# kxhit/vMAP

Measured on AMD Instinct MI355X. Metric: training rays/sec (all objects) per step, higher is better.
Workload: dtype f32 I/O, masters, accumulation; matrix operands split into bf16 planes: forward 6 products (~2^-24, float32-equivalent), backward 3 (~2^-16)

## Files before the change

### vmap_amd/csrc/k_s32.hip

```cpp
#include "launch.h"
#include "split_kernels.h"

namespace vl {

namespace {
template <bool BWD, bool MULTI, bool STAMPS, bool W3, bool B6 = false, bool PV = false, bool OL = false>
int main_v(const vk::StepArgs& a, hipStream_t st) {
    auto kern = vk::step_main_s32<BWD, MULTI, STAMPS, W3, B6, PV, OL>;
    if (int rc = ensure_dynamic_lds(reinterpret_cast<const void*>(kern), vk::Img32s::LDS_BYTES, "step_main_s32")) return rc;
    const int grid = a.xcd_affine ? 8 * ((a.n_obj + 7) / 8) * a.NW : a.n_obj * a.NW;
    VL_LAUNCH_MAIN(kern, dim3(grid), dim3(vk::kWG), vk::Img32s::LDS_BYTES, st, a);
    return launched("step_main_s32");
}
#ifdef VMAPSTEP_AB
template <bool MULTI, bool W3, bool B6>
int main_of(const vk::StepArgs& a, hipStream_t st) {
    auto kern = vk::step_main_s32_of<MULTI, W3, B6>;
    if (int rc = ensure_dynamic_lds(reinterpret_cast<const void*>(kern), vk::Img32s::LDS_BYTES, "step_main_s32")) return rc;
    const int grid = a.xcd_affine ? 8 * ((a.n_obj + 7) / 8) * a.NW : a.n_obj * a.NW;
    VL_LAUNCH_MAIN(kern, dim3(grid), dim3(vk::kWG), vk::Img32s::LDS_BYTES, st, a);
    return launched("step_main_s32");
}
template <bool MULTI, bool STAMPS, bool W3, bool B6>
int main_ob(const vk::StepArgs& a, hipStream_t st) {
    auto kern = vk::step_main_s32_ob<MULTI, STAMPS, W3, B6>;
    if (int rc = ensure_dynamic_lds(reinterpret_cast<const void*>(kern), vk::Img32s::LDS_BYTES, "step_main_s32")) return rc;
    const int grid = a.xcd_affine ? 8 * ((a.n_obj + 7) / 8) * a.NW : a.n_obj * a.NW;
    VL_LAUNCH_MAIN(kern, dim3(grid), dim3(vk::kWG), vk::Img32s::LDS_BYTES, st, a);
    return launched("step_main_s32");
}
#endif
template <bool BWD, bool STAMPS>
int main_bs(const vk::StepArgs& a, hipStream_t st) {
    const bool multi = a.NW < a.NG;
#ifdef VMAPSTEP_AB
    if (a.ab_flags & 8) {
        if constexpr (BWD) {
            if (!(a.ab_flags & 7)) {
                if constexpr (STAMPS) {
                    if (!a.weights_bf16 && !a.bwd6 && !multi) return main_ob<false, true, true, false>(a, st);
                } else {
                    if (a.weights_bf16) return multi ? main_ob<true, false, false, false>(a, st) : main_ob<false, false, false, false>(a, st);
                    if (a.bwd6) return multi ? main_ob<true, false, true, true>(a, st) : main_ob<false, false, true, true>(a, st);
                    return multi ? main_ob<true, false, true, false>(a, st) : main_ob<false, false, true, false>(a, st);
                }
            }
        }
        return fail(-2, "tuning.ws_flags bit 6 (the former backward of step_main_s32): training steps without bit 3, 4 or 5; phase stamps with float32 weights, the three-product backward and one pass per workgroup only");
    }
    if (a.ab_flags & 4) {
        if constexpr (BWD && !STAMPS) {
            if (!(a.ab_flags & 3)) {
                if (a.weights_bf16) return multi ? main_of<true, false, false>(a, st) : main_of<false, false, false>(a, st);
                if (a.bwd6) return multi ? main_of<true, true, true>(a, st) : main_of<false, true, true>(a, st);
                return multi ? main_of<true, true, false>(a, st) : main_of<false, true, false>(a, st);
            }
        }
        return fail(-2, "tuning.ws_flags bit 5 (the former front of step_main_s32): training steps without phase stamps, bit 3 or bit 4");
    }
    if (a.ab_flags & 2) {
        if constexpr (BWD && !STAMPS) {
            if (!a.bwd6 && !(a.ab_flags & 1)) {
                if (a.weights_bf16) return multi ? main_v<true, true, false, false, false, false, true>(a, st) : main_v<true, false, false, false, false, false, true>(a, st);
                return multi ? main_v<true, true, false, true, false, false, true>(a, st) : main_v<true, false, false, true, false, false, true>(a, st);
            }
        }
        return fail(-2, "tuning.ws_flags bit 4 (the former load order of step_main_s32): training steps without phase stamps, bit 3 or the six-product backward");
    }
// ... 36 lines not shown
```

### vmap_amd/csrc/split_kernels.h

```cpp
#pragma once
#ifndef VS_ABL
#define VS_ABL 0
#endif
#include "step_kernels.h"
#include "wave_reduce.h"
#ifndef VS_FRONT_PARTS
#define VS_FRONT_PARTS 15
#endif
#ifndef VS_BACK_PARTS
#define VS_BACK_PARTS 7
#endif

#ifndef VS_ABL
#define VS_ABL 0
#endif
#if VS_ABL & 2
#define VS_BWD_BARRIER() do { } while (0)
#else
#define VS_BWD_BARRIER() __syncthreads()
#endif

namespace vk {

using wv::u32x2;
using wv::u32x4;

struct Img32s {
    static constexpr int PIT_IN = 208, PIT_M = 80, PIT_CAT = 272, PIT_C = 176;
    static constexpr int O_IN = 0, O_M1 = O_IN + 32 * PIT_IN, O_CAT = O_M1 + 32 * PIT_M, O_M2 = O_CAT + 32 * PIT_CAT,
                         O_C = O_M2 + 32 * PIT_M, PLANE = O_C + 32 * PIT_C;
    static constexpr int P_HI = 0, P_MID = PLANE, SMALL = 2 * PLANE, SMALL_BYTES = 2048, P_LO = SMALL + SMALL_BYTES,
                         END = P_LO + PLANE, BYTES = (END + 4095) / 4096 * 4096;
    static constexpr int ROUNDS = BYTES / 4096;
    static constexpr int ELEMS = PLANE / 2;
    static constexpr int B_M1 = 0, B_M2 = 32, W_A = 64, W_OC = 96, B_A = 192, B_OC = 196, PE_B = 200, SMALL_N = 208;
    static constexpr int G_PEB = SMALL_N, VEC_N = SMALL_N + 66 + 6;
    static constexpr int TILE = 32 * Lds32::TP * 4;
    static constexpr int TPL = TILE / 2;
    static constexpr int TPIT = 72;
    static constexpr int SCR = BYTES;
    static constexpr int STG = SCR;
    static constexpr int STG_BYTES = 2 * kWaves * TILE, kWavesTiles = kWaves * 2 * TILE;
    static constexpr int VEC = SCR + kWaves * 2 * TILE;
// ... 683 lines not shown
            } else {
                const unsigned pm = wv::pack_bf16(wv::after(ra[i], accB[0]), rb[i]);
                hm[i] = pm;
                hl[i] = wv::pack_bf16(ra[i] - bf_lo(pm), rb[i] - bf_hi(pm));
            }
        }
        wv::sched_fence();
    }
}

template <bool BIG>
__device__ __forceinline__ void octave_sincos(float a0, float (&s)[6], float (&c)[6]) {
    if (BIG) sincosf(a0, &s[0], &c[0]);
    else sincos_f32(a0, s[0], c[0]);
#pragma unroll
    for (int f = 1; f < 6; ++f) {
        const float t = s[f - 1] + s[f - 1];
        s[f] = t * c[f - 1];
        c[f] = fmaf(-t, s[f - 1], 1.0f);
    }
}

__device__ __forceinline__ void stage_put_s(float* stage, const f32x16& acc, int wave, int p31, int hi) {
    if (!(VS_ABL & 9)) stage_put(stage, acc, wave, p31, hi);
    else if (VS_ABL & 8) {
#pragma unroll
        for (int r = 0; r < 16; ++r) asm volatile("" ::"v"(acc[r]));
    }
}
__device__ __forceinline__ void stage_get_s(float (&q)[4], const float* stage, int wave, int p31, int hi) {
    if (!(VS_ABL & 9)) stage_get(q, stage, wave, p31, hi);
}

template <bool BWD, bool MULTI, bool STAMPS, bool W3, bool B6 = false, bool PV = false, bool OL = false, bool OF = false, bool OB = false>
__device__ __forceinline__ void step_main_s32_body(const StepArgs& a) {
    static_assert(!B6 || (W3 && BWD), "six-product backward: float32 weights, training instantiations");
    constexpr int OLD = OL ? 7 : VS_LOADS_OLD;
    constexpr int FP = OF ? 0 : VS_FRONT_PARTS;
    constexpr int BP = OB ? 0 : VS_BACK_PARTS;
    constexpr bool TC = (BP & 1) != 0, TD = (BP & 2) != 0, ZC = (BP & 4) != 0 && !MULTI;
    using I = Img32s;
    using F = Flat32;
    constexpr int H = 32;
    char* lds = reinterpret_cast<char*>(wv::lds_base());
    const char* W = lds;
    const float* SM = reinterpret_cast<const float*>(lds + I::SMALL);
    const int tid = threadIdx.x, lane = tid & 63, wave = tid >> 6, p31 = lane & 31, hi = lane >> 5;
    float* Gv = reinterpret_cast<float*>(lds + I::VEC) + wave * I::VEC_N;
    int obj, wgo;
    if (a.xcd_affine) {
        const int slot = blockIdx.x >> 3;
        const int og = slot / a.NW;
        obj = og * 8 + (blockIdx.x & 7);
        wgo = slot - og * a.NW;
        if (obj >= a.n_obj) return;
    } else {
        obj = blockIdx.x / a.NW;
        wgo = blockIdx.x - obj * a.NW;
    }
    unsigned* tmark = STAMPS && a.timing ? a.timing + ((long long)blockIdx.x * kWaves + wave) * kMarks : nullptr;
#define VS_MARK(i) do { if constexpr (STAMPS) { if (tmark && lane == 0) tmark[i] = wv::clock32(); } } while (0)
    VS_MARK(0);
    if (BWD) {
        for (int i = tid; i < kWaves * I::VEC_N; i += kWG) reinterpret_cast<float*>(lds + I::VEC)[i] = 0.0f;
    }
    float* loss_cells = reinterpret_cast<float*>(lds + I::LOSS);
    if (tid < kWaves * 4) loss_cells[tid] = 0.0f;
    float* out = a.part_grad + ((long long)(obj * a.NW + wgo)) * a.PP;
    float qacc[12][4];
#pragma unroll
    for (int b = 0; b < 12; ++b) {
#pragma unroll
        for (int i = 0; i < 4; ++i) qacc[b][i] = 0.0f;
// ... 221 lines not shown
            row[2] = sigmoidf_acc(r1);
            row[3] = sigmoidf_acc(r2);
        }
        if (BWD) {
            toF_put(reinterpret_cast<float*>(scrX), h4, p31, hi);
            toF_put(reinterpret_cast<float*>(scrD), hc, p31, hi);
        }
    }
    VS_MARK(4);
    if (!(VS_ABL & 65536)) __syncthreads();
    VS_MARK(5);
    {
        const StepArgs& al = wv::kernarg_late(a);
        if constexpr (OLD & 2) {
        if (!(VS_ABL & 2048))
        composite_phase<BWD>(al, cb, loss_cells, obj, ray0, nrays, wave, lane, tid,
                             (VS_ABL & 1024) ? rays_meta : finish_ray_meta(al, obj, rays_meta));
        } else if (!(VS_ABL & 2048)) composite_phase<BWD>(al, cb, loss_cells, obj, ray0, nrays, wave, lane, tid, rays_meta);
    }
    if (!(VS_ABL & 65536)) __syncthreads();
    VS_MARK(6);
    if (BWD) {
    float d_raw, d_c0, d_c1, d_c2;
    {
        const float* row = cb + pt * 8;
        d_raw = row[0]; d_c0 = row[1]; d_c1 = row[2]; d_c2 = row[3];
    }
    constexpr int DM = !W3 ? 0 : B6 ? 2 : 1, NA = kDpropMM(DM), NPW = !W3 ? 1 : B6 ? 3 : 2, NPB = B6 ? 3 : 2, NDW = kDwMM(B6), NDB = kDwDbMM(B6);
    unsigned dF[24];
    float dproj[11];
#pragma unroll
    for (int i = 0; i < 11; ++i) dproj[i] = 0.0f;
    unsigned dch[8], dcm[8], dcl[8], d4h[8], d4m[8], d4l[8];
    {
        float h4F[16], hcF[16];
        toF_get(h4F, reinterpret_cast<const float*>(scrX), p31, hi);
        toF_get(hcF, reinterpret_cast<const float*>(scrD), p31, hi);
        float ga = 0.0f, g0 = 0.0f, g1 = 0.0f, g2 = 0.0f, sa = 0.0f, s0 = 0.0f, s1 = 0.0f, s2 = 0.0f;
#pragma unroll
        for (int r = 0; r < 16; ++r) {
            const float* row = cbw + (r + 16 * hi) * 8;
            const float da = row[0], q0 = row[1], q1 = row[2], q2 = row[3];
            ga = fmaf(da, h4F[r], ga);
            g0 = fmaf(q0, hcF[r], g0); g1 = fmaf(q1, hcF[r], g1); g2 = fmaf(q2, hcF[r], g2);
            sa += da; s0 += q0; s1 += q1; s2 += q2;
        }
        ga += wv::swap_half(ga); g0 += wv::swap_half(g0); g1 += wv::swap_half(g1); g2 += wv::swap_half(g2);
        sa += wv::swap_half(sa); s0 += wv::swap_half(s0); s1 += wv::swap_half(s1); s2 += wv::swap_half(s2);
        if (hi == 0) {
            if constexpr (ZC) {
                Gv[I::W_A + p31] = 0.0f + ga;
                Gv[I::W_OC + p31] = 0.0f + g0;
                Gv[I::W_OC + H + p31] = 0.0f + g1;
                Gv[I::W_OC + 2 * H + p31] = 0.0f + g2;
                if (p31 == 0) {
                    Gv[I::B_A] = 0.0f + sa;
                    Gv[I::B_OC + 0] = 0.0f + s0;
                    Gv[I::B_OC + 1] = 0.0f + s1;
                    Gv[I::B_OC + 2] = 0.0f + s2;
                }
            } else {
                Gv[I::W_A + p31] += ga;
                Gv[I::W_OC + p31] += g0;
                Gv[I::W_OC + H + p31] += g1;
                Gv[I::W_OC + 2 * H + p31] += g2;
                if (p31 == 0) {
                    Gv[I::B_A] += sa;
                    Gv[I::B_OC + 0] += s0;
                    Gv[I::B_OC + 1] += s1;
                    Gv[I::B_OC + 2] += s2;
                }
            }
        }
        float dcp[16];
#pragma unroll
        for (int r = 0; r < 16; ++r) {
            const int j = phi(r, hi);
            const float v = SM[I::W_OC + j] * d_c0 + SM[I::W_OC + H + j] * d_c1 + SM[I::W_OC + 2 * H + j] * d_c2;
            dcp[r] = wv::opaque(hc[r]) > 0.0f ? v : 0.0f;
        }
        split_planes<16, NPB>(dcp, dch, dcm, dcl);
    }
    f32x16 acc2, accb;
    FinState fs;
    unsigned wA[24], wB[24], xA[24], xB[24];
    unsigned d3h[8], d3m[8], d3l[8], d2h[8], d2m[8], d2l[8], d1h[8], d1m[8], d1l[8], dF3[24], dF1[24];
    const auto nothing = [](int) {};
    const auto dproj_add = [&](int d, float v, float c) {
        if constexpr (TD) { const float sum = dproj[d] + v * c; dproj[d] = wv::after(sum, sum); }
        else dproj[d] += v * c;
    };
#define VS_FIN(KIND, K, QI, STG, OW, OB, BLK, NC)                                                                             \
    [&](int i) {                                                                                                              \
        if (i == 0) fin_chunk<KIND, K, MULTI>(0, fs, qacc[QI], STG, OW, OB, BLK, NC, wave, p31, hi);                          \
        if (i == NA - 3) fin_chunk<KIND, K, MULTI>(1, fs, qacc[QI], STG, OW, OB, BLK, NC, wave, p31, hi);                     \
    }
    const SelOps SEL = sel_ops(p31, hi);
    wt_get<I::PIT_C, NPW>(wA, W + I::O_C, 0, TL);
    toF_mm3<4, NPB>(dF, dch, dcm, dcl, SEL);
    toF_mm3<4, NPB>(xA, h4h, h4m, h4l, SEL);
    wt_get<I::PIT_C, NPW>(wB, W + I::O_C, 2, TL);
#pragma unroll
    for (int r = 0; r < 16; ++r) acc2[r] = SM[I::W_A + phi(r, hi)] * d_raw;
    mm_dprop_il<DM>(acc2, wA, dch, dcm, dcl, nothing);
    toF_mm3<4, NPB>(xB, e2h, e2m, e2l, SEL);
    zero_acc(acc);
    mm_dw_il<false, B6>(acc, accb, dF, xA, [&](int i) {
#pragma unroll
        for (int j = i * 8 / NDW; j < (i + 1) * 8 / NDW; ++j) mask_split_pair<NPB>(j, acc2, h4h, d4h, d4m, d4l, acc[0]);
    });
    wt_get<I::PIT_C, NPW>(wA, W + I::O_C, 4, TL);
    VS_BWD_BARRIER();
    zero_acc(acc2);
    mm_dprop_il<DM>(acc2, wB, dch, dcm, dcl, [&](int i) { if (i == NA - 1) stage_put_s(stg0, acc, wave, p31, hi); });
    toF_mm3<2, NPB>(xA, e2h + 8, e2m + 8, e2l + 8, SEL);
    wt_get<I::PIT_M, NPW>(wB, W + I::O_M2, 0, TL);
    zero_acc(acc);
    mm_dw_il<false, B6>(acc, accb, dF, xB, [&](int i) {
        if (i < 4) {
#pragma unroll
            for (int r = 4 * i; r < 4 * i + 4; ++r) dproj_add(r >> 1, wv::after(acc2[r], acc[0]), cfac[r >> 1][4 + (r & 1)]);
        }
    });
    VS_BWD_BARRIER();
    zero_acc(acc2);
    {
        auto fin = VS_FIN(0, H + kEmb2, 0, stg0, out + F::W_C, nullptr, 0, 32);
        mm_dprop_il<DM>(acc2, wA, dch, dcm, dcl, [&](int i) { fin(i); if (i == NA - 1) stage_put_s(stg1, acc, wave, p31, hi); });
    }
    toF_mm3<4, NPB>(xB, h3h, h3m, h3l, SEL);
    wt_get<I::PIT_CAT, NPW>(wA, W + I::O_CAT, 0, TL);
    zero_acc(acc);
    mm_dw_il<false, B6>(acc, accb, dF, xA, [&](int i) {
        if (i < 3) {
#pragma unroll
            for (int r = 2 * i; r < 2 * i + 2; ++r) dproj_add(8 + (r >> 1), wv::after(acc2[r], acc[0]), cfac[8 + (r >> 1)][4 + (r & 1)]);
        }
    });
    toF_mm3<4, NPB>(dF, d4h, d4m, d4l, SEL);
    VS_BWD_BARRIER();
    VS_MARK(7);
    zero_acc(acc2);
    {
// ... 15 lines not shown
    zero_acc(acc2);
    {
        auto fin = VS_FIN(2, H + kEmb2, 2, stg0, out + F::W_C + H, out + F::B_C, 1, kEmb2);
        mm_dprop_il<DM>(acc2, wA, d3h, d3m, d3l, [&](int i) { fin(i); if (i == NA - 1) stage_put_s(stg1, acc, wave, p31, hi); });
    }
    toF_mm3<4, NPB>(xB, h1h, h1m, h1l, SEL);
    wt_get<I::PIT_CAT, NPW>(wA, W + I::O_CAT, 2, TL);
    zero_acc(acc);
    mm_dw_il<false, B6>(acc, accb, dF3, xA, [&](int i) {
#pragma unroll
        for (int j = i * 8 / NDW; j < (i + 1) * 8 / NDW; ++j) mask_split_pair<NPB>(j, acc2, h2h, d2h, d2m, d2l, acc[0]);
    });
    toF_mm3<4, NPB>(dF, d2h, d2m, d2l, SEL);
    VS_BWD_BARRIER();
    VS_MARK(9);
    zero_acc(acc2);
    {
        auto fin = VS_FIN(0, H, 3, stg1, out + F::W_M2, nullptr, 0, 32);
        mm_dprop_il<DM>(acc2, wB, d2h, d2m, d2l, [&](int i) { fin(i); if (i == NA - 1) stage_put_s(stg0, acc, wave, p31, hi); });
    }
    toF_mm3<4, NPB>(xA, e1h, e1m, e1l, SEL);
    wt_get<I::PIT_IN, NPW>(wB, W + I::O_IN, 0, TL);
    zero_acc(acc);
    zero_acc(accb);
    mm_dw_il<true, B6>(acc, accb, dF, xB, [&](int i) {
#pragma unroll
        for (int j = i * 8 / NDB; j < (i + 1) * 8 / NDB; ++j) mask_split_pair<NPB, TC>(j, acc2, h1h, d1h, d1m, d1l, i < NDW ? acc[0] : accb[0]);
    });
    bias_sums_put<ZC>(Gv + I::B_M1, accb, p31, hi);
    toF_mm3<4, NPB>(dF1, d1h, d1m, d1l, SEL);
    VS_BWD_BARRIER();
    VS_MARK(10);
    f32x16 de;
#pragma unroll
    for (int blk = 0; blk < 3; ++blk) {
        unsigned (&xc)[24] = (blk & 1) ? xB : xA;
        unsigned (&xn)[24] = (blk & 1) ? xA : xB;
        zero_acc(de);
        if (blk == 0) {
            auto fin = VS_FIN(0, H + kEmb1, 4, stg0, out + F::W_CAT, nullptr, 0, 32);
            mm_dprop_il<DM>(de, wA, d3h, d3m, d3l, [&](int i) { fin(i); if (i == NA - 1) stage_put_s(stg1, acc, wave, p31, hi); });
        } else {
            auto fin = VS_FIN(1, H + kEmb1, 6 + blk - 1, stg0, out + F::W_CAT + H, out + F::B_CAT, blk - 1, kEmb1);
            mm_dprop_il<DM>(de, wA, d3h, d3m, d3l, [&](int i) { fin(i); if (i == NA - 1) stage_put_s(stg1, acc, wave, p31, hi); });
        }
        if (blk < 2) {
            wt_get<I::PIT_CAT, NPW>(wA, W + I::O_CAT, 2 + 2 * (blk + 1), TL);
            toF_mm3<4, NPB>(xn, e1h + 8 * (blk + 1), e1m + 8 * (blk + 1), e1l + 8 * (blk + 1), SEL);
        }
        zero_acc(acc);
        mm_dw_il<false, B6>(acc, accb, dF3, xc, nothing);
        VS_BWD_BARRIER();
        if (blk == 0) {
            auto fin = VS_FIN(0, H, 5, stg1, out + F::W_M1, nullptr, 0, 32);
            mm_dprop_il<DM>(de, wB, d1h, d1m, d1l, [&](int i) { fin(i); if (i == NA - 1) stage_put_s(stg0, acc, wave, p31, hi); });
        } else {
            auto fin = VS_FIN(1, kEmb1, 9 + blk - 1, stg1, out + F::W_IN, out + F::B_IN, blk - 1, kEmb1);
            mm_dprop_il<DM>(de, wB, d1h, d1m, d1l, [&](int i) { fin(i); if (i == NA - 1) stage_put_s(stg0, acc, wave, p31, hi); });
        }
        if (blk < 2) wt_get<I::PIT_IN, NPW>(wB, W + I::O_IN, 2 * (blk + 1), TL);
        zero_acc(acc);
        mm_dw_il<false, B6>(acc, accb, dF1, xc, [&](int i) {
            if (i < 4) {
#pragma unroll
                for (int r = 4 * i; r < 4 * i + 4; ++r) {
                    const int R = 16 * blk + r;
                    if (R < 44) dproj_add(R >> 2, wv::after(de[r], acc[0]), cfac[R >> 2][R & 3]);
                }
            }
        });
        VS_BWD_BARRIER();
    }
    VS_MARK(11);
    VS_MARK(12);
    {
        fin_chunk<1, H + kEmb1, MULTI>(0, fs, qacc[8], stg0, out + F::W_CAT + H, out + F::B_CAT, 2, kEmb1, wave, p31, hi);
        stage_put_s(stg1, acc, wave, p31, hi);
        fin_chunk<1, H + kEmb1, MULTI>(1, fs, qacc[8], stg0, out + F::W_CAT + H, out + F::B_CAT, 2, kEmb1, wave, p31, hi);
        float keep[3] = {0.0f, 0.0f, 0.0f};
        if constexpr (PV) {
#pragma unroll
            for (int i = 0; i < 11; ++i) {
#pragma unroll
                for (int j = 0; j < 3; ++j) {
                    const int v = 3 * i + j;
                    const float sum = wv::half_sum32_hi_row(dproj[i] * t[j]);
                    keep[v >> 4] = (lane & 15) == (v & 15) ? sum : keep[v >> 4];
                }
            }
        } else {
#pragma unroll
            for (int sl = 0; sl < 2; ++sl)
                keep[sl] = wv::half_dots32_scatter16([&](int c, float& d, float& tt) { const int v = 16 * sl + c; d = dproj[v / 3]; tt = t[v % 3]; }, lane);
            keep[2] = wv::half_dot32_hi_row(dproj[10], t[2], lane);
        }
        if (lane & 16) {
#pragma unroll
            for (int sl = 0; sl < 3; ++sl) {
                const int v = 16 * sl + (lane & 15);
                if (v < 33) {
                    if constexpr (ZC) Gv[I::G_PEB + 36 * hi + v] = 0.0f + keep[sl];
                    else Gv[I::G_PEB + 36 * hi + v] += keep[sl];
                }
            }
        }
        VS_BWD_BARRIER();
        finish_block_s<1, kEmb1, MULTI>(qacc[11], stg1, out + F::W_IN, out + F::B_IN, 2, kEmb1, wave, p31, hi);
    }
#undef VS_FIN
    VS_MARK(13);
    }
    if (!MULTI) break;
    }
    __syncthreads();
    VS_MARK(14);
    if (tid == 0) {
        float* pl = a.part_loss + (obj * a.NW + wgo) * 4;
#pragma unroll
        for (int k = 0; k < 3; ++k)
            pl[k] = (loss_cells[k] + loss_cells[4 + k]) + (loss_cells[8 + k] + loss_cells[12 + k]);
        pl[3] = 0.0f;
    }
    if (!BWD) return;

    if (MULTI) {
        int col; bool bias;
// ... 15 lines not shown
    }
    for (int sv = tid; sv < I::VEC_N; sv += kWG) {
        const float* v = reinterpret_cast<const float*>(lds + I::VEC) + sv;
        const float g = (v[0] + v[I::VEC_N]) + (v[2 * I::VEC_N] + v[3 * I::VEC_N]);
        int o = -1;
        if (sv >= I::G_PEB) {
            const int x = sv - I::G_PEB, hf = x >= 36 ? 1 : 0, vv = x - 36 * hf, i = vv / 3;
            if (vv < 33 && i < (hf ? 10 : 11)) o = F::PE_B + 3 * (hf ? 11 + i : i) + (vv - 3 * i);
        } else
        if (sv < I::B_M2) o = F::B_M1 + (sv - I::B_M1);
        else if (sv < I::W_A) o = F::B_M2 + (sv - I::B_M2);
        else if (sv < I::W_OC) o = F::W_A + (sv - I::W_A);
        else if (sv < I::B_A) o = F::W_OC + (sv - I::W_OC);
        else if (sv == I::B_A) o = F::B_A;
        else if (sv >= I::B_OC && sv < I::B_OC + 3) o = F::B_OC + (sv - I::B_OC);
        if (o >= 0) out[o] = g;
    }
    VS_MARK(15);
#undef VS_MARK
}

template <bool BWD, bool MULTI, bool STAMPS, bool W3, bool B6 = false, bool PV = false, bool OL = false>
__global__ __launch_bounds__(kWG, 1) void step_main_s32(const StepArgs a) {
    step_main_s32_body<BWD, MULTI, STAMPS, W3, B6, PV, OL>(a);
}
template <bool MULTI, bool W3, bool B6>
__global__ __launch_bounds__(kWG, 1) void step_main_s32_of(const StepArgs a) {
    step_main_s32_body<true, MULTI, false, W3, B6, false, false, true>(a);
}
template <bool MULTI, bool STAMPS, bool W3, bool B6>
__global__ __launch_bounds__(kWG, 1) void step_main_s32_ob(const StepArgs a) {
    step_main_s32_body<true, MULTI, STAMPS, W3, B6, false, false, false, true>(a);
}

}
```

### vmap_amd/csrc/step_plan.h

```cpp
#pragma once
#include <algorithm>
#include <cmath>
#include <cstddef>
#include <cstdint>
#include <cstring>

#include "../../include/vmapstep.h"
#include "wide_kernels.h"
#include "wpair_kernels.h"

namespace vl {

int fail(int code, const char* fmt, ...);

constexpr size_t kAlign = 256;
constexpr int kMaxFrameSteps = 256;
inline size_t align_up(size_t x) { return (x + kAlign - 1) / kAlign * kAlign; }
constexpr const char* kMeasurementOnly = "this kernel form ships in the measurement build only (tests/tools/libvmapstep_ab.so: phase stamps and A/B forms no automatic plan launches)";

inline const vmapstep_tuning& tuning_of(const vmapstep_shape* sh) {
    static const vmapstep_tuning kAutoTuning = {0, VMAPSTEP_KERNEL_AUTO, 0, 0};
    return (sh && sh->tuning) ? *sh->tuning : kAutoTuning;
}

// ... 38 lines not shown
};

inline int check_shape(const vmapstep_shape* sh, int max_steps) {
    if (!sh) return fail(VMAPSTEP_ERR_ARGUMENT, "shape is null");
    if (sh->n_obj < 1 || sh->rays < 1 || sh->samples < 1 || max_steps < 1)
        return fail(VMAPSTEP_ERR_ARGUMENT, "bad shape n=%d R=%d S=%d steps=%d", sh->n_obj, sh->rays, sh->samples, max_steps);
    return VMAPSTEP_OK;
}

inline int plan_family(const vmapstep_shape* sh, bool measurement_build, Family& fam) {
    if (sh->hidden < 32 || sh->hidden > 256 || sh->hidden % 32 != 0)
        return fail(VMAPSTEP_ERR_UNSUPPORTED, "hidden=%d: supported widths are multiples of 32 up to 256", sh->hidden);
    if (sh->weight_dtype != VMAPSTEP_WEIGHTS_F32 && sh->weight_dtype != VMAPSTEP_WEIGHTS_BF16)
        return fail(VMAPSTEP_ERR_UNSUPPORTED, "weight_dtype=%d", sh->weight_dtype);
    if (sh->samples > vk::kMaxPts)
        return fail(VMAPSTEP_ERR_UNSUPPORTED, "samples=%d > %d", sh->samples, vk::kMaxPts);
    const vmapstep_tuning& tun = tuning_of(sh);
    const int force = tun.kernel, H = sh->hidden;
    if (force < VMAPSTEP_KERNEL_AUTO || (force > VMAPSTEP_KERNEL_WP && force != VMAPSTEP_KERNEL_S32_BWD6)) return fail(VMAPSTEP_ERR_ARGUMENT, "tuning.kernel=%d", force);
    fam = H != 32 ? kGen : force == VMAPSTEP_KERNEL_H32_F32 ? kH32 : force == VMAPSTEP_KERNEL_S32_BWD6 ? kS32Bwd6 : kS32;
    if (force == VMAPSTEP_KERNEL_S32_BWD6 && (H != 32 || sh->weight_dtype != VMAPSTEP_WEIGHTS_F32))
        return fail(VMAPSTEP_ERR_UNSUPPORTED, "VMAPSTEP_KERNEL_S32_BWD6: hidden 32 with float32 weights");
    if (H != 32 && H % 128 == 0 && force != VMAPSTEP_KERNEL_GEN && sh->samples <= vk::kWideTile) {
        const int gw = std::min(vk::kWideTile / sh->samples, sh->rays);
        const long long tiles = (long long)sh->n_obj * ((sh->rays + gw - 1) / gw);
        if (force == VMAPSTEP_KERNEL_WIDE4 || (force == VMAPSTEP_KERNEL_AUTO && tiles <= 256)) fam = kWide;
    }
    if ((H == 128 || H == 64) && sh->samples <= vk::ImgWs<4>::kPts) {
        if (force == VMAPSTEP_KERNEL_AUTO) fam = H == 64 ? kWp : kWs;
        else if (force == VMAPSTEP_KERNEL_WS1) fam = kWs;
        else if (force == VMAPSTEP_KERNEL_WP) fam = kWp;
    }
    if (H == 256 && sh->samples <= 32 && (force == VMAPSTEP_KERNEL_AUTO || force == VMAPSTEP_KERNEL_WS1)) fam = kWs;
    if (!measurement_build && split32(fam) && (tun.ws_flags & (8 | 16 | 32 | 64)))
        return fail(VMAPSTEP_ERR_UNSUPPORTED, "%s", kMeasurementOnly);
    if ((force == VMAPSTEP_KERNEL_WS1 || force == VMAPSTEP_KERNEL_WP) && !block_native_rows(fam))
        return fail(VMAPSTEP_ERR_UNSUPPORTED, "VMAPSTEP_KERNEL_WS1 / _WP: hidden 64 / 128 with at most 64 samples per ray (_WS1 also hidden 256 with at most 32)");
    return VMAPSTEP_OK;
}

inline int plan_rounds(const vmapstep_shape* sh, bool measurement_build, Plan& pl) {
    const vmapstep_tuning& tun = tuning_of(sh);
    const Family fam = pl.family;
    const int cap = fam == kWs && sh->hidden == 256 ? 32 : round_points(fam, 2);
    if (sh->samples > cap) return fail(VMAPSTEP_ERR_UNSUPPORTED, "samples=%d > %d", sh->samples, cap);
    pl.G = round_points(fam, 2) / sh->samples;
    pl.tiles = 2;
    if (fam == kWs) {
        const int g1 = 32 / sh->samples, g2 = pl.G, g3 = 96 / sh->samples;
        const bool autoplan = tun.workgroups_per_object <= 0;
        auto rounds = [&](int g) { return g >= 1 ? (long long)sh->n_obj * ((sh->rays + std::min(g, sh->rays) - 1) / std::min(g, sh->rays)) : (1LL << 40); };
        if (sh->hidden == 256) { pl.G = g1; pl.tiles = 1; }
        else if (sh->hidden == 128 && (tun.ws_flags & 2)) { pl.G = g3; pl.tiles = 3; }
        else if (autoplan && !(tun.ws_flags & 1) && rounds(g1) <= 256) { pl.G = g1; pl.tiles = 1; }
        else if (autoplan && sh->hidden == 128 && !(tun.ws_flags & 4) && rounds(g2) > 256 && rounds(g3) <= 256) { pl.G = g3; pl.tiles = 3; }
    }
    if (pl.G > sh->rays) pl.G = sh->rays;
    pl.NG = (sh->rays + pl.G - 1) / pl.G;
    const int wg_slots = (fam == kWp && sh->hidden == 64) ? 512 : 256;
    int nw = tun.workgroups_per_object > 0 ? tun.workgroups_per_object : wg_slots / sh->n_obj;
    if (nw < 1) nw = 1;
    if (nw > pl.NG) nw = pl.NG;
    if (block_native_rows(fam) && tun.workgroups_per_object <= 0) {
        const int per = (pl.NG + nw - 1) / nw;
        nw = (pl.NG + per - 1) / per;
    }
    pl.NW = nw;
// ... 26 lines not shown
    pl.off_tab_wt = o; o += wt_image(fam) ? table : 0;
    pl.off_row_tab = o; o += block_native_rows(fam) ? align_up((size_t)pl.PR * sizeof(int)) : 0;
    pl.off_pgrad = o; o += align_up(wgs * pl.PR * sizeof(float));
    pl.off_wimg = o; o += align_up((size_t)sh->n_obj * image);
    pl.off_scratch = o; o += scratch ? align_up(wgs * scratch) : 0;
    pl.off_flags = o; o += align_up((size_t)kMaxFrameSteps * 4 * sizeof(int));
    pl.off_stats = o; o += align_up((size_t)max_steps * sh->n_obj * 4 * sizeof(float));
    pl.total = o;
    return VMAPSTEP_OK;
}

inline int make_plan(const vmapstep_shape* sh, int max_steps, bool measurement_build, const Layout& L, Plan& pl) {
    if (int rc = check_shape(sh, max_steps)) return rc;
    if (int rc = plan_family(sh, measurement_build, pl.family)) return rc;
    if (int rc = plan_rounds(sh, measurement_build, pl)) return rc;
    return plan_sections(sh, max_steps, L, pl);
}

inline int main_xcd_affine(Family fam, int n_obj, int NW) {
    return fam == kWp ? (n_obj >= 8 ? 1 : 0) : (hidden32(fam) && ((n_obj + 7) / 8) * NW <= 32) ? 1 : 0;
}
inline int main_workgroups(const vk::StepArgs& a) { return (a.xcd_affine ? 8 * ((a.n_obj + 7) / 8) : a.n_obj) * a.NW; }

inline void fill_step_plan(vk::StepArgs& a, const vmapstep_shape* sh, const Plan& pl, const Layout& L) {
    std::memset(&a, 0, sizeof(a));
    a.n_obj = sh->n_obj; a.R = sh->rays; a.S = sh->samples;
    a.G = pl.G; a.NG = pl.NG; a.NW = pl.NW; a.PP = L.PP; a.PR = pl.PR; a.tiles = pl.tiles;
    a.xcd_affine = main_xcd_affine(pl.family, sh->n_obj, pl.NW);
    a.hidden = sh->hidden;
    a.weights_bf16 = sh->weight_dtype == VMAPSTEP_WEIGHTS_BF16 ? 1 : 0;
    a.wide = step_args_wide(pl.family);
    a.split = split32(pl.family) ? 1 : 0;
    a.bwd6 = pl.family == kS32Bwd6 ? 1 : 0;
    a.ab_flags = split32(pl.family) ? ((tuning_of(sh).ws_flags & 8) ? 1 : 0) | ((tuning_of(sh).ws_flags & 16) ? 2 : 0) | ((tuning_of(sh).ws_flags & 32) ? 4 : 0) | ((tuning_of(sh).ws_flags & 64) ? 8 : 0) : 0;
}
inline void fill_step_workspace(vk::StepArgs& a, const Plan& pl, char* ws) {
    auto ints = [&](bool have, size_t off) { return have ? reinterpret_cast<int*>(ws + off) : nullptr; };
    a.stats = reinterpret_cast<float*>(ws + pl.off_stats);
    a.flags = reinterpret_cast<int*>(ws + pl.off_flags);
    a.part_loss = reinterpret_cast<float*>(ws + pl.off_ploss);
    a.img_tab = ints(image_table(pl.family), pl.off_imgtab);
    a.tab_wt = ints(wt_image(pl.family), pl.off_tab_wt);
    a.row_tab = ints(block_native_rows(pl.family), pl.off_row_tab);
    a.part_grad = reinterpret_cast<float*>(ws + pl.off_pgrad);
    a.wimg = reinterpret_cast<float*>(ws + pl.off_wimg);
    a.gen_scratch = reinterpret_cast<float*>(ws + pl.off_scratch);
}
inline void fill_step_args(vk::StepArgs& a, const vmapstep_shape* sh, const Plan& pl, const Layout& L,
                           const vmapstep_params* params, const vmapstep_tensor* pe_scale, const vmapstep_batch* b,
                           int64_t ray0, float cw, float ow, char* ws) {
    fill_step_plan(a, sh, pl, L);
    fill_step_workspace(a, pl, ws);
    for (int t = 0; t < VMAPSTEP_NUM_FC; ++t) a.fc[t] = {params->fc[t].ptr, params->fc[t].obj_stride};
    a.pe_B = {params->pe_B.ptr, params->pe_B.obj_stride};
    a.pe_scale = {pe_scale->ptr, pe_scale->obj_stride};
    if (b->pcs) {
        a.pcs = b->pcs + ray0 * b->pcs_stride[1];
        a.pcs_so = b->pcs_stride[0]; a.pcs_sr = b->pcs_stride[1]; a.pcs_ss = b->pcs_stride[2]; a.pcs_sc = b->pcs_stride[3];
    } else {
        a.ray_o = b->ray_o + ray0 * b->ray_o_stride[1];
        a.ro_so = b->ray_o_stride[0]; a.ro_sr = b->ray_o_stride[1]; a.ro_sc = b->ray_o_stride[2];
        a.ray_d = b->ray_d + ray0 * b->ray_d_stride[1];
        a.rd_so = b->ray_d_stride[0]; a.rd_sr = b->ray_d_stride[1]; a.rd_sc = b->ray_d_stride[2];
        a.center = b->center; a.ce_so = b->center_stride;
    }
    a.z = b->z + ray0 * b->z_stride[1];
    a.z_so = b->z_stride[0]; a.z_sr = b->z_stride[1]; a.z_ss = b->z_stride[2];
// ... 82 lines not shown
```

### vmap_amd/csrc/wave_reduce.h

```cpp
#pragma once
#include <wave_ops.h>

namespace wv {

constexpr int rs_slot(int c) {
    return (((c >> 0) ^ (c >> 2)) & 1) | ((((c >> 1) ^ (c >> 2)) & 1) << 1) | ((((c >> 2) ^ (c >> 3)) & 1) << 2) | (((c >> 3) & 1) << 3);
}

#ifdef __HIP__
#define WV_RS_FN __device__ __forceinline__
template <int CTRL>
WV_RS_FN float rs_partner(float x, int) {
    return __uint_as_float(__builtin_amdgcn_update_dpp(__float_as_uint(x), __float_as_uint(x), CTRL, 0xf, 0xf, true));
}
WV_RS_FN float rs_row_below(float x, int) {
    const unsigned u = __float_as_uint(x);
    const auto r = __builtin_amdgcn_permlane16_swap(u, u, false, false);
    return __uint_as_float(r[0]);
}
WV_RS_FN float rs_row_below15(float x, int) {
    return __uint_as_float(__builtin_amdgcn_update_dpp(__float_as_uint(x), __float_as_uint(x), 0x142, 0xA, 0xF, false));
}
#else
#define WV_RS_FN inline
// ... 20 lines not shown
        }
    }
#pragma unroll
    for (int i = 0; i < N / 2; ++i) a[i] = o[i];
}

WV_RS_FN float half_dot32_hi_row(float d, float t, int lane) {
    float x = rs_first(d, t, lane);
    x += rs_partner<0x4E>(x, lane);
    x += rs_partner<0x141>(x, lane);
    x += rs_partner<0x140>(x, lane);
    return x + rs_row_below15(x, lane);
}

template <class F>
WV_RS_FN float half_dots32_scatter16(F&& val, int lane) {
    float a[16];
#pragma unroll
    for (int c = 0; c < 16; ++c) {
        float d, t;
        val(c, d, t);
        a[rs_slot(c)] = rs_first(d, t, lane);
    }
    rs_step<16, 0x4E>(a, (((lane >> 1) ^ (lane >> 2)) & 1) != 0, lane);
    rs_step<8, 0x141>(a, (((lane >> 2) ^ (lane >> 3)) & 1) != 0, lane);
    rs_step<4, 0x140>(a, ((lane >> 3) & 1) != 0, lane);
    const bool k1 = ((lane ^ (lane >> 2)) & 1) != 0;
    const float mine = k1 ? a[1] : a[0];
    const float from_class0 = rs_partner<0xB1>(a[1], lane);
    const float for_above = k1 ? from_class0 : a[0];
    return mine + rs_row_below(for_above, lane);
}

#undef WV_RS_FN

}
```

Measured before the change: 91.21 million.

## Interleave head gradients and first butterfly reduction into backward matrix phases

Moves the head-layer gradient accumulation (per-row FMAs over cbw rows) into the callbacks of the dprop and dW matrix loops, and splits the first half-dot butterfly reduction into steps spread across the last block's matrix phases. The aim is to hide the serial scalar and DPP work under the matrix instruction latency instead of running it as separate exposed phases. Both are enabled by default through the new back-parts bits. An A/B flag keeps the old placement for measurement. The cost is more register pressure and a more complex schedule.

```diff
diff --git a/vmap_amd/csrc/k_s32.hip b/vmap_amd/csrc/k_s32.hip
--- a/vmap_amd/csrc/k_s32.hip
+++ b/vmap_amd/csrc/k_s32.hip
@@ -29,11 +29,33 @@
     VL_LAUNCH_MAIN(kern, dim3(grid), dim3(vk::kWG), vk::Img32s::LDS_BYTES, st, a);
     return launched("step_main_s32");
 }
+template <bool MULTI, bool STAMPS, bool W3, bool B6>
+int main_oh(const vk::StepArgs& a, hipStream_t st) {
+    auto kern = vk::step_main_s32_oh<MULTI, STAMPS, W3, B6>;
+    if (int rc = ensure_dynamic_lds(reinterpret_cast<const void*>(kern), vk::Img32s::LDS_BYTES, "step_main_s32")) return rc;
+    const int grid = a.xcd_affine ? 8 * ((a.n_obj + 7) / 8) * a.NW : a.n_obj * a.NW;
+    VL_LAUNCH_MAIN(kern, dim3(grid), dim3(vk::kWG), vk::Img32s::LDS_BYTES, st, a);
+    return launched("step_main_s32");
+}
 #endif
 template <bool BWD, bool STAMPS>
 int main_bs(const vk::StepArgs& a, hipStream_t st) {
     const bool multi = a.NW < a.NG;
 #ifdef VMAPSTEP_AB
+    if (a.ab_flags & 16) {
+        if constexpr (BWD) {
+            if (!(a.ab_flags & 15)) {
+                if constexpr (STAMPS) {
+                    if (!a.weights_bf16 && !a.bwd6 && !multi) return main_oh<false, true, true, false>(a, st);
+                } else {
+                    if (a.weights_bf16) return multi ? main_oh<true, false, false, false>(a, st) : main_oh<false, false, false, false>(a, st);
+                    if (a.bwd6) return multi ? main_oh<true, false, true, true>(a, st) : main_oh<false, false, true, true>(a, st);
+                    return multi ? main_oh<true, false, true, false>(a, st) : main_oh<false, false, true, false>(a, st);
+                }
+            }
+        }
+        return fail(-2, "tuning.ws_flags bit 7 (the former place of step_main_s32's head gradients and first B_layer butterfly): training steps without bit 3, 4, 5 or 6; phase stamps with float32 weights, the three-product backward and one pass per workgroup only");
+    }
     if (a.ab_flags & 8) {
         if constexpr (BWD) {
             if (!(a.ab_flags & 7)) {
diff --git a/vmap_amd/csrc/split_kernels.h b/vmap_amd/csrc/split_kernels.h
--- a/vmap_amd/csrc/split_kernels.h
+++ b/vmap_amd/csrc/split_kernels.h
@@ -8,7 +8,7 @@
 #define VS_FRONT_PARTS 15
 #endif
 #ifndef VS_BACK_PARTS
-#define VS_BACK_PARTS 7
+#define VS_BACK_PARTS 31
 #endif
 
 #ifndef VS_ABL
@@ -758,13 +758,14 @@
     if (!(VS_ABL & 9)) stage_get(q, stage, wave, p31, hi);
 }
 
-template <bool BWD, bool MULTI, bool STAMPS, bool W3, bool B6 = false, bool PV = false, bool OL = false, bool OF = false, bool OB = false>
+template <bool BWD, bool MULTI, bool STAMPS, bool W3, bool B6 = false, bool PV = false, bool OL = false, bool OF = false, bool OB = false, bool OH = false>
 __device__ __forceinline__ void step_main_s32_body(const StepArgs& a) {
     static_assert(!B6 || (W3 && BWD), "six-product backward: float32 weights, training instantiations");
     constexpr int OLD = OL ? 7 : VS_LOADS_OLD;
     constexpr int FP = OF ? 0 : VS_FRONT_PARTS;
-    constexpr int BP = OB ? 0 : VS_BACK_PARTS;
+    constexpr int BP = OB ? 0 : OH ? (VS_BACK_PARTS & 7) : VS_BACK_PARTS;
     constexpr bool TC = (BP & 1) != 0, TD = (BP & 2) != 0, ZC = (BP & 4) != 0 && !MULTI;
+    constexpr bool HG = (BP & 8) != 0 && !(MULTI && B6), HB = (BP & 16) != 0 && !PV && !(MULTI && B6);
     using I = Img32s;
     using F = Flat32;
     constexpr int H = 32;
@@ -1052,19 +1053,19 @@
 #pragma unroll
     for (int i = 0; i < 11; ++i) dproj[i] = 0.0f;
     unsigned dch[8], dcm[8], dcl[8], d4h[8], d4m[8], d4l[8];
-    {
-        float h4F[16], hcF[16];
-        toF_get(h4F, reinterpret_cast<const float*>(scrX), p31, hi);
-        toF_get(hcF, reinterpret_cast<const float*>(scrD), p31, hi);
-        float ga = 0.0f, g0 = 0.0f, g1 = 0.0f, g2 = 0.0f, sa = 0.0f, s0 = 0.0f, s1 = 0.0f, s2 = 0.0f;
-#pragma unroll
-        for (int r = 0; r < 16; ++r) {
-            const float* row = cbw + (r + 16 * hi) * 8;
-            const float da = row[0], q0 = row[1], q1 = row[2], q2 = row[3];
-            ga = fmaf(da, h4F[r], ga);
-            g0 = fmaf(q0, hcF[r], g0); g1 = fmaf(q1, hcF[r], g1); g2 = fmaf(q2, hcF[r], g2);
-            sa += da; s0 += q0; s1 += q1; s2 += q2;
-        }
+    float h4F[16], hcF[16];
+    float ga = 0.0f, g0 = 0.0f, g1 = 0.0f, g2 = 0.0f, sa = 0.0f, s0 = 0.0f, s1 = 0.0f, s2 = 0.0f;
+    wv::f32x4 hrow;
+    const auto head_row_get = [&](int r) { hrow = *reinterpret_cast<const wv::f32x4*>(cbw + (r + 16 * hi) * 8); };
+    const auto head_row = [&](int r) {
+        const float da = hrow[0], q0 = hrow[1], q1 = hrow[2], q2 = hrow[3];
+        if (r + 1 < 16) head_row_get(r + 1);
+        const float na = fmaf(da, h4F[r], ga), n0 = fmaf(q0, hcF[r], g0), n1 = fmaf(q1, hcF[r], g1), n2 = fmaf(q2, hcF[r], g2);
+        ga = wv::after(na, na); g0 = wv::after(n0, n0); g1 = wv::after(n1, n1); g2 = wv::after(n2, n2);
+        const float ma = sa + da, m0 = s0 + q0, m1 = s1 + q1, m2 = s2 + q2;
+        sa = wv::after(ma, ma); s0 = wv::after(m0, m0); s1 = wv::after(m1, m1); s2 = wv::after(m2, m2);
+    };
+    const auto head_cells = [&](float ga, float g0, float g1, float g2, float sa, float s0, float s1, float s2) {
         ga += wv::swap_half(ga); g0 += wv::swap_half(g0); g1 += wv::swap_half(g1); g2 += wv::swap_half(g2);
         sa += wv::swap_half(sa); s0 += wv::swap_half(s0); s1 += wv::swap_half(s1); s2 += wv::swap_half(s2);
         if (hi == 0) {
@@ -1092,6 +1093,53 @@
                 }
             }
         }
+    };
+    {
+        if constexpr (HG) {
+            toF_get(h4F, reinterpret_cast<const float*>(scrX), p31, hi);
+            toF_get(hcF, reinterpret_cast<const float*>(scrD), p31, hi);
+            head_row_get(0);
+        } else {
+            float h4F[16], hcF[16];
+            toF_get(h4F, reinterpret_cast<const float*>(scrX), p31, hi);
+            toF_get(hcF, reinterpret_cast<const float*>(scrD), p31, hi);
+            float ga = 0.0f, g0 = 0.0f, g1 = 0.0f, g2 = 0.0f, sa = 0.0f, s0 = 0.0f, s1 = 0.0f, s2 = 0.0f;
+#pragma unroll
+            for (int r = 0; r < 16; ++r) {
+                const float* row = cbw + (r + 16 * hi) * 8;
+                const float da = row[0], q0 = row[1], q1 = row[2], q2 = row[3];
+                ga = fmaf(da, h4F[r], ga);
+                g0 = fmaf(q0, hcF[r], g0); g1 = fmaf(q1, hcF[r], g1); g2 = fmaf(q2, hcF[r], g2);
+                sa += da; s0 += q0; s1 += q1; s2 += q2;
+            }
+            ga += wv::swap_half(ga); g0 += wv::swap_half(g0); g1 += wv::swap_half(g1); g2 += wv::swap_half(g2);
+            sa += wv::swap_half(sa); s0 += wv::swap_half(s0); s1 += wv::swap_half(s1); s2 += wv::swap_half(s2);
+            if (hi == 0) {
+                if constexpr (ZC) {
+                    Gv[I::W_A + p31] = 0.0f + ga;
+                    Gv[I::W_OC + p31] = 0.0f + g0;
+                    Gv[I::W_OC + H + p31] = 0.0f + g1;
+                    Gv[I::W_OC + 2 * H + p31] = 0.0f + g2;
+                    if (p31 == 0) {
+                        Gv[I::B_A] = 0.0f + sa;
+                        Gv[I::B_OC + 0] = 0.0f + s0;
+                        Gv[I::B_OC + 1] = 0.0f + s1;
+                        Gv[I::B_OC + 2] = 0.0f + s2;
+                    }
+                } else {
+                    Gv[I::W_A + p31] += ga;
+                    Gv[I::W_OC + p31] += g0;
+                    Gv[I::W_OC + H + p31] += g1;
+                    Gv[I::W_OC + 2 * H + p31] += g2;
+                    if (p31 == 0) {
+                        Gv[I::B_A] += sa;
+                        Gv[I::B_OC + 0] += s0;
+                        Gv[I::B_OC + 1] += s1;
+                        Gv[I::B_OC + 2] += s2;
+                    }
+                }
+            }
+        }
         float dcp[16];
 #pragma unroll
         for (int r = 0; r < 16; ++r) {
@@ -1122,13 +1170,24 @@
     wt_get<I::PIT_C, NPW>(wB, W + I::O_C, 2, TL);
 #pragma unroll
     for (int r = 0; r < 16; ++r) acc2[r] = SM[I::W_A + phi(r, hi)] * d_raw;
-    mm_dprop_il<DM>(acc2, wA, dch, dcm, dcl, nothing);
+    constexpr int HRA = 2 * NA < 16 ? 2 * NA : 16, HRB = 16 - HRA;
+    mm_dprop_il<DM>(acc2, wA, dch, dcm, dcl, [&](int i) {
+        if constexpr (HG) {
+#pragma unroll
+            for (int r = HRA * i / NA; r < HRA * (i + 1) / NA; ++r) head_row(r);
+        }
+    });
     toF_mm3<4, NPB>(xB, e2h, e2m, e2l, SEL);
     zero_acc(acc);
     mm_dw_il<false, B6>(acc, accb, dF, xA, [&](int i) {
 #pragma unroll
-        for (int j = i * 8 / NDW; j < (i + 1) * 8 / NDW; ++j) mask_split_pair<NPB>(j, acc2, h4h, d4h, d4m, d4l, acc[0]);
+        for (int j = i * 8 / NDW; j < (i + 1) * 8 / NDW; ++j) mask_split_pair<NPB, HG>(j, acc2, h4h, d4h, d4m, d4l, acc[0]);
+        if constexpr (HG) {
+#pragma unroll
+            for (int r = HRA + (i * HRB + NDW - 1) / NDW; r < HRA + ((i + 1) * HRB + NDW - 1) / NDW; ++r) head_row(r);
+        }
     });
+    if constexpr (HG) head_cells(ga, g0, g1, g2, sa, s0, s1, s2);
     wt_get<I::PIT_C, NPW>(wA, W + I::O_C, 4, TL);
     VS_BWD_BARRIER();
     zero_acc(acc2);
@@ -1210,6 +1269,13 @@
     VS_BWD_BARRIER();
     VS_MARK(10);
     f32x16 de;
+    wv::HalfDots32Scatter16 bf0;
+    constexpr int NBS = NA - 1 + NDW;
+    const auto bf0_steps = [&](int s) {
+#pragma unroll
+        for (int k = wv::HalfDots32Scatter16::kSteps * s / NBS; k < wv::HalfDots32Scatter16::kSteps * (s + 1) / NBS; ++k)
+            bf0.step(k, [&](int c, float& d, float& tt) { d = dproj[c / 3]; tt = t[c % 3]; }, lane);
+    };
 #pragma unroll
     for (int blk = 0; blk < 3; ++blk) {
         unsigned (&xc)[24] = (blk & 1) ? xB : xA;
@@ -1220,14 +1286,18 @@
             mm_dprop_il<DM>(de, wA, d3h, d3m, d3l, [&](int i) { fin(i); if (i == NA - 1) stage_put_s(stg1, acc, wave, p31, hi); });
         } else {
             auto fin = VS_FIN(1, H + kEmb1, 6 + blk - 1, stg0, out + F::W_CAT + H, out + F::B_CAT, blk - 1, kEmb1);
-            mm_dprop_il<DM>(de, wA, d3h, d3m, d3l, [&](int i) { fin(i); if (i == NA - 1) stage_put_s(stg1, acc, wave, p31, hi); });
+            mm_dprop_il<DM>(de, wA, d3h, d3m, d3l, [&](int i) {
+                fin(i);
+                if (i == NA - 1) stage_put_s(stg1, acc, wave, p31, hi);
+                if constexpr (HB) { if (blk == 2 && i != NA - 3) bf0_steps(i < NA - 3 ? i : i - 1); }
+            });
         }
         if (blk < 2) {
             wt_get<I::PIT_CAT, NPW>(wA, W + I::O_CAT, 2 + 2 * (blk + 1), TL);
             toF_mm3<4, NPB>(xn, e1h + 8 * (blk + 1), e1m + 8 * (blk + 1), e1l + 8 * (blk + 1), SEL);
         }
         zero_acc(acc);
-        mm_dw_il<false, B6>(acc, accb, dF3, xc, nothing);
+        mm_dw_il<false, B6>(acc, accb, dF3, xc, [&](int i) { if constexpr (HB) { if (blk == 2) bf0_steps(NA - 1 + i); } });
         VS_BWD_BARRIER();
         if (blk == 0) {
             auto fin = VS_FIN(0, H, 5, stg1, out + F::W_M1, nullptr, 0, 32);
@@ -1268,8 +1338,9 @@
             }
         } else {
 #pragma unroll
-            for (int sl = 0; sl < 2; ++sl)
+            for (int sl = HB ? 1 : 0; sl < 2; ++sl)
                 keep[sl] = wv::half_dots32_scatter16([&](int c, float& d, float& tt) { const int v = 16 * sl + c; d = dproj[v / 3]; tt = t[v % 3]; }, lane);
+            if constexpr (HB) keep[0] = bf0.sum;
             keep[2] = wv::half_dot32_hi_row(dproj[10], t[2], lane);
         }
         if (lane & 16) {
@@ -1351,5 +1422,9 @@
 __global__ __launch_bounds__(kWG, 1) void step_main_s32_ob(const StepArgs a) {
     step_main_s32_body<true, MULTI, STAMPS, W3, B6, false, false, false, true>(a);
 }
-
-}
+template <bool MULTI, bool STAMPS, bool W3, bool B6>
+__global__ __launch_bounds__(kWG, 1) void step_main_s32_oh(const StepArgs a) {
+    step_main_s32_body<true, MULTI, STAMPS, W3, B6, false, false, false, false, true>(a);
+}
+
+}
diff --git a/vmap_amd/csrc/step_plan.h b/vmap_amd/csrc/step_plan.h
--- a/vmap_amd/csrc/step_plan.h
+++ b/vmap_amd/csrc/step_plan.h
@@ -94,7 +94,7 @@
         else if (force == VMAPSTEP_KERNEL_WP) fam = kWp;
     }
     if (H == 256 && sh->samples <= 32 && (force == VMAPSTEP_KERNEL_AUTO || force == VMAPSTEP_KERNEL_WS1)) fam = kWs;
-    if (!measurement_build && split32(fam) && (tun.ws_flags & (8 | 16 | 32 | 64)))
+    if (!measurement_build && split32(fam) && (tun.ws_flags & (8 | 16 | 32 | 64 | 128)))
         return fail(VMAPSTEP_ERR_UNSUPPORTED, "%s", kMeasurementOnly);
     if ((force == VMAPSTEP_KERNEL_WS1 || force == VMAPSTEP_KERNEL_WP) && !block_native_rows(fam))
         return fail(VMAPSTEP_ERR_UNSUPPORTED, "VMAPSTEP_KERNEL_WS1 / _WP: hidden 64 / 128 with at most 64 samples per ray (_WS1 also hidden 256 with at most 32)");
@@ -187,7 +187,7 @@
     a.wide = step_args_wide(pl.family);
     a.split = split32(pl.family) ? 1 : 0;
     a.bwd6 = pl.family == kS32Bwd6 ? 1 : 0;
-    a.ab_flags = split32(pl.family) ? ((tuning_of(sh).ws_flags & 8) ? 1 : 0) | ((tuning_of(sh).ws_flags & 16) ? 2 : 0) | ((tuning_of(sh).ws_flags & 32) ? 4 : 0) | ((tuning_of(sh).ws_flags & 64) ? 8 : 0) : 0;
+    a.ab_flags = split32(pl.family) ? ((tuning_of(sh).ws_flags & 8) ? 1 : 0) | ((tuning_of(sh).ws_flags & 16) ? 2 : 0) | ((tuning_of(sh).ws_flags & 32) ? 4 : 0) | ((tuning_of(sh).ws_flags & 64) ? 8 : 0) | ((tuning_of(sh).ws_flags & 128) ? 16 : 0) : 0;
 }
 inline void fill_step_workspace(vk::StepArgs& a, const Plan& pl, char* ws) {
     auto ints = [&](bool have, size_t off) { return have ? reinterpret_cast<int*>(ws + off) : nullptr; };
diff --git a/vmap_amd/csrc/wave_reduce.h b/vmap_amd/csrc/wave_reduce.h
--- a/vmap_amd/csrc/wave_reduce.h
+++ b/vmap_amd/csrc/wave_reduce.h
@@ -76,6 +76,41 @@
     return mine + rs_row_below(for_above, lane);
 }
 
+struct HalfDots32Scatter16 {
+    static constexpr int kSteps = 16 + 8 + 4 + 2 + 1;
+    float a[16], b[8], c[4], e[2], sum;
+
+    template <int CTRL>
+    static WV_RS_FN float piece(const float* v, int p, bool key, int lane) {
+        const int q = p >> 1, b0 = p & 1;
+        const float lo = v[4 * q + b0], up = v[4 * q + 2 + b0];
+        const float keep = key ? up : lo;
+        const float send = key ? lo : up;
+        const float s = keep + rs_partner<CTRL>(send, lane);
+        return after(s, s);
+    }
+    template <class F>
+    WV_RS_FN void step(int k, F&& val, int lane) {
+        if (k < 16) {
+            float d, t;
+            val(k, d, t);
+            const float s = rs_first(d, t, lane);
+            a[rs_slot(k)] = after(s, s);
+        } else if (k < 24) b[k - 16] = piece<0x4E>(a, k - 16, (((lane >> 1) ^ (lane >> 2)) & 1) != 0, lane);
+        else if (k < 28) c[k - 24] = piece<0x141>(b, k - 24, (((lane >> 2) ^ (lane >> 3)) & 1) != 0, lane);
+        else if (k < 30) e[k - 28] = piece<0x140>(c, k - 28, ((lane >> 3) & 1) != 0, lane);
+        else {
+            const bool k1 = ((lane ^ (lane >> 2)) & 1) != 0;
+            const float e0 = e[0], e1 = e[1];
+            const float mine = k1 ? e1 : e0;
+            const float from_class0 = rs_partner<0xB1>(e1, lane);
+            const float for_above = k1 ? from_class0 : e0;
+            const float s = mine + rs_row_below(for_above, lane);
+            sum = after(s, s);
+        }
+    }
+};
+
 #undef WV_RS_FN
 
 }
```

Result: no change. 91.88 million (median of 6 runs) (+0.7%).
